# Total-RD/pymgrid

Measured on AMD Instinct MI355X. Metric: microgrid env-steps/sec, higher is better.
Workload: dtype f64

## Files before the change

pymgrid_amd/csrc/mgx_fused.hip:

```cpp
#include "mgx_kernels.hpp"

#ifndef MGX_FUSED_PART
#error "compile with -DMGX_FUSED_PART=<0..MGX_FUSED_PARTS-1>"
#endif

#if MGX_FUSED_PART == 0
#define MGX_PART_FLAGS(X) X(0) X(1) X(2) X(4)
#elif MGX_FUSED_PART == 1
#define MGX_PART_FLAGS(X) X(3) X(5)
#elif MGX_FUSED_PART == 2
#define MGX_PART_FLAGS(X) X(6) X(7)
#elif MGX_FUSED_PART == 3
#define MGX_PART_FLAGS(X) X(14)
#elif MGX_FUSED_PART == 4
#define MGX_PART_FLAGS(X) X(15)
#elif MGX_FUSED_PART == 5
#define MGX_PART_FLAGS(X)
#else
#error "MGX_FUSED_PART out of range"
#endif

#define MGX_CAT2(a, b) a##b
#define MGX_CAT(a, b) MGX_CAT2(a, b)

#if MGX_FUSED_PART == 5
namespace mgx {
#define MGX_STATIC_LAYOUTS(X) \
    X(7, 2, 2, 1, 1, 1) X(7, 2, 2, 2, 1, 1) X(7, 2, 2, 2, 2, 2) X(7, 1, 2, 1, 1, 1) X(7, 1, 2, 2, 1, 1) X(7, 2, 1, 1, 1, 1) X(7, 1, 1, 2, 1, 1) \
    X(3, 2, 2, 0, 1, 1) X(3, 2, 1, 0, 1, 1) X(3, 1, 2, 0, 1, 1) X(6, 0, 2, 1, 1, 1) X(6, 0, 2, 2, 1, 1) X(6, 0, 1, 2, 1, 1) \
                           \
    X(7, 3, 3, 1, 1, 1) X(7, 3, 2, 1, 1, 1) X(7, 2, 3, 1, 1, 1) X(3, 3, 3, 0, 1, 1) X(6, 0, 3, 1, 1, 1)
bool launch_step_k_multi_static(const MultiStaticLaunch &L)
{
#define X(FV, G, B, R, LD, PV)                                                                                                           \
    if (L.flags == FV && L.ng == G && L.nb == B && L.nr == R && L.nl == LD && L.np == PV) {                                             \
        using CT = CountsCT<G, B, R, LD, PV>;                                                                                          \
        step_k_multi_small_kernel<FV, CT, CT::slots><<<L.blocks, BLOCK_MULTI, 0, L.stream>>>(*L.k, L.actions, L.t, L.K, L.normalized, L.out); \
        return true;                                                                                                                    \
    }
    MGX_STATIC_LAYOUTS(X)
#undef X
    return false;
}
bool launch_rollout_multi_static(const MultiStaticRollout &L)
{
#define X(FV, G, B, R, LD, PV)                                                                                                           \
    if (L.flags == FV && L.ng == G && L.nb == B && L.nr == R && L.nl == LD && L.np == PV) {                                             \
        using CT = CountsCT<G, B, R, LD, PV>;                                                                                          \
        rollout_multi_small_kernel<FV, CT, CT::slots><<<L.blocks, BLOCK_MULTI, 0, L.stream>>>(*L.k, L.lists, L.n_lists, L.list_len,     \
                                                                                             L.ids, L.per_step, L.t, L.K, L.out);      \
        return true;                                                                                                                    \
    }
    MGX_STATIC_LAYOUTS(X)
#undef X
    return false;
}
}
#else

namespace mgx {

template <int F, bool RC, bool FC>
constexpr int ring_depth()
{
    if (FC) return RC ? ((F & F_GRID) ? 8 : MGX_RING_RICH) : MGX_RING;
    return (F & F_GRID) ? 4 : (RC ? 4 : MGX_RING);
}

template <int F>
static void step_k_dispatch(const FusedLaunch &L)
{
#define MGX_STEP_K(AT, RC, FC) step_k_kernel<F, ring_depth<F, RC, FC>(), AT, RC, FC><<<L.blocks, BLOCK_K, 0, L.stream>>>( \
        *L.k, (const AT *)L.actions, L.t, L.K, L.normalized, L.out, L.gpb)
    if (L.act_f32) {
        if (L.fact) { if (L.rich) MGX_STEP_K(float, true, true); else MGX_STEP_K(float, false, true); }
        else { if (L.rich) MGX_STEP_K(float, true, false); else MGX_STEP_K(float, false, false); }
    } else {
        if (L.fact) { if (L.rich) MGX_STEP_K(double, true, true); else MGX_STEP_K(double, false, true); }
        else { if (L.rich) MGX_STEP_K(double, true, false); else MGX_STEP_K(double, false, false); }
    }
#undef MGX_STEP_K
}

template <int F>
static void rollout_dispatch(const FusedLaunch &L)
{
#define MGX_ROLLOUT(PS, RC, FC) rollout_kernel<F, (F & F_GRID) ? 4 : MGX_RING_ROLLOUT, PS, RC, FC><<<L.blocks, BLOCK_K, 0, L.stream>>>( \
        *L.k, *L.tab, L.ids, L.t, L.K, L.out, L.gpb)
    if (L.fact) {
        if (L.per_step) { if (L.rich) MGX_ROLLOUT(true, true, true); else MGX_ROLLOUT(true, false, true); }
        else { if (L.rich) MGX_ROLLOUT(false, true, true); else MGX_ROLLOUT(false, false, true); }
    } else {
        if (L.per_step) { if (L.rich) MGX_ROLLOUT(true, true, false); else MGX_ROLLOUT(true, false, false); }
        else { if (L.rich) MGX_ROLLOUT(false, true, false); else MGX_ROLLOUT(false, false, false); }
    }
#undef MGX_ROLLOUT
}

bool MGX_CAT(launch_step_k_p, MGX_FUSED_PART)(const FusedLaunch &L)
{
    switch (L.flags) {
#define X(FV) case FV: step_k_dispatch<FV>(L); return true;
        MGX_PART_FLAGS(X)
#undef X
        default: return false;
    }
}

bool MGX_CAT(launch_rollout_p, MGX_FUSED_PART)(const FusedLaunch &L)
{
    switch (L.flags) {
#define X(FV) case FV: rollout_dispatch<FV>(L); return true;
        MGX_PART_FLAGS(X)
#undef X
        default: return false;
    }
}

}
#endif
```

pymgrid_amd/csrc/mgx_kernels.hpp:

```cpp
#pragma once
#include "mgx_core.hpp"

#include <type_traits>

namespace mgx {

#ifndef MGX_BLOCK
#define MGX_BLOCK 128
#endif
constexpr int BLOCK = MGX_BLOCK;
#ifndef MGX_RING
#define MGX_RING 8
#endif
#ifndef MGX_RING_RICH
#define MGX_RING_RICH 16
#endif
#ifndef MGX_BLOCK_K
#define MGX_BLOCK_K 256
#endif
constexpr int BLOCK_K = MGX_BLOCK_K;
#ifndef MGX_RING_ROLLOUT
#define MGX_RING_ROLLOUT 8
#endif

#ifndef MGX_HOT_NT
#define MGX_HOT_NT 1
#endif
#ifndef MGX_ACT_NT
#define MGX_ACT_NT 0
#endif
#ifndef MGX_OUT_NT
#define MGX_OUT_NT 0
#endif
#ifndef MGX_ROWS_NT
#define MGX_ROWS_NT 1
#endif
#ifndef MGX_STATE_NT
#define MGX_STATE_NT 1
#endif
#ifndef MGX_ROWS_TILE
#define MGX_ROWS_TILE 1
#endif
constexpr int ROW_TILE_MAX_D = 12;
__host__ __device__ inline bool step_rows_tiled(const KArgs &a, const void *obs)
{
    return MGX_ROWS_TILE && obs != nullptr && a.H == 0 && !a.obs_state_only && a.obs_dim <= ROW_TILE_MAX_D;
}

template <int F, typename OT>
__device__ __forceinline__ void observe_row_h0_tiled(const KArgs &a, int64_t i, int32_t t_next, const Params &p, const State &s,
                                                     OT *__restrict__ obs, int32_t pm, OT *tile)
{
    const int lane = threadIdx.x & 63;
    const int32_t D = a.obs_dim;
    observe_row_h0<F>(a, i, t_next, p, s, tile + lane * D, pm);
    __builtin_amdgcn_wave_barrier();
    typedef OT vec2 __attribute__((ext_vector_type(2)));
    typedef OT vec4 __attribute__((ext_vector_type(4)));
    OT *out = obs + (i - lane) * D;
    const int32_t total = 64 * D;
    if constexpr (sizeof(OT) == 8) {
        if ((reinterpret_cast<uintptr_t>(out) & 15) == 0) {
            for (int32_t e = 2 * lane; e < total; e += 128) {
                const vec2 v = *reinterpret_cast<const vec2 *>(tile + e);
#if MGX_ROWS_NT
                __builtin_nontemporal_store(v, reinterpret_cast<vec2 *>(out + e));
#else
                *reinterpret_cast<vec2 *>(out + e) = v;
#endif
            }
        } else {
            for (int32_t e = lane; e < total; e += 64) out[e] = tile[e];
        }
    } else {
        if ((total & 3) == 0 && (reinterpret_cast<uintptr_t>(out) & 15) == 0) {
            for (int32_t e = 4 * lane; e < total; e += 256) {
                const vec4 v = *reinterpret_cast<const vec4 *>(tile + e);
#if MGX_ROWS_NT
                __builtin_nontemporal_store(v, reinterpret_cast<vec4 *>(out + e));
#else
                *reinterpret_cast<vec4 *>(out + e) = v;
#endif
            }
        } else {
            for (int32_t e = 2 * lane; e < total; e += 128) {
                const vec2 v = *reinterpret_cast<const vec2 *>(tile + e);
                *reinterpret_cast<vec2 *>(out + e) = v;
            }
        }
    }
}

template <int F>
__device__ __forceinline__ void store_step_obs(const KArgs &a, void *__restrict__ obs, int64_t i, int32_t t_next, const Params &p,
                                               const State &s, int32_t pm = 0,
                                               double *tile = nullptr)
{
    constexpr int NSTATE = 4 * ((F & F_GENSET) != 0) + 2 * ((F & F_BATTERY) != 0);
// ... 92 lines not shown

template <int F, bool EP = false>
__global__ __launch_bounds__(BLOCK) void step_kernel(const KArgs a, const void *__restrict__ actions, int32_t t,
                                                     int normalized, double *__restrict__ reward,
                                                     uint8_t *__restrict__ done, void *__restrict__ obs,
                                                     double *__restrict__ log)
{
    t = resolve_t(a, t);
    extern __shared__ __attribute__((aligned(16))) double row_tiles[];
    const int64_t i = (int64_t)a.g0 + (int64_t)blockIdx.x * BLOCK + threadIdx.x;
    if (i < a.g1) step_body<F, EP>(a, actions, t, normalized, reward, done, obs, log, i, row_tiles + (threadIdx.x >> 6) * (64 * ROW_TILE_MAX_D));
    advance_counter_in_kernel(a, 1);
}

template <int F>
__global__ __launch_bounds__(BLOCK) void check_kernel(const KArgs a, const void *__restrict__ actions, int32_t t, int normalized,
                                                      uint32_t *__restrict__ violations)
{
    t = resolve_t(a, t);
    const int64_t i = (int64_t)a.g0 + (int64_t)blockIdx.x * BLOCK + threadIdx.x;
    if (i >= a.g1) return;
    Params p; State s; Inputs in; Outputs o; Derived d;
    load_state<F>(a.c, i, true, s);
    load_params<F>(a.c, i, p);
    derive<F>(p, d);
    const int64_t row = series_row(a, i, t);
    if (a.act_f32) load_inputs<F>(a.c, (const float *)actions, a.N, i, row, in, a.pm_pitch);
    else load_inputs<F>(a.c, (const double *)actions, a.N, i, row, in, a.pm_pitch);
    step_core<F>(p, d, s, in, normalized != 0, false, false, o);
    violations[i] = o.violations;
}

struct FusedOut {
    double *reward;
    uint8_t *done;
    double *soc_trace;
    uint32_t *status_trace;
    double *ret_acc;
    double *log;
};

template <typename AT>
struct RawInputs {
    AT a_goal, a_gen, a_bat, a_grid;
    double load, pv, g_pimp, g_pexp, g_co2, g_stat;
};

template <int F, typename AT>
__device__ __forceinline__ Inputs widen(const RawInputs<AT> &r)
{
    Inputs in;
    if constexpr (F & F_GENSET) { in.a_goal = (double)r.a_goal; in.a_gen = (double)r.a_gen; }
    if constexpr (F & F_BATTERY) in.a_bat = (double)r.a_bat;
    if constexpr (F & F_GRID) {
        in.a_grid = (double)r.a_grid;
        in.g_pimp = r.g_pimp; in.g_pexp = r.g_pexp; in.g_co2 = r.g_co2; in.g_stat = r.g_stat;
    }
    in.load = r.load; in.pv = r.pv;
    return in;
}

template <int F, typename AT>
__device__ __forceinline__ void load_inputs_at(const AT *__restrict__ act, const double *__restrict__ lts,
                                               const double *__restrict__ pts, const double *__restrict__ gts,
                                               int64_t N, int64_t i, int64_t off, RawInputs<AT> &in)
{
    constexpr int A = 2 * ((F & F_GENSET) != 0) + ((F & F_BATTERY) != 0) + ((F & F_GRID) != 0);
    const AT *a = act + off * A;
    int k = 0;
    if constexpr (F & F_GENSET) { in.a_goal = a[k]; in.a_gen = a[k + 1]; k += 2; }
    if constexpr (F & F_BATTERY) { in.a_bat = a[k]; k += 1; }
    if constexpr (F & F_GRID) { in.a_grid = a[k]; k += 1; }
    in.load = lts[off];
    in.pv = pts[off];
    if constexpr (F & F_GRID) {
        const double *g = gts + (4 * off - 3 * i);
        in.g_pimp = g[0]; in.g_pexp = g[N]; in.g_co2 = g[2 * N]; in.g_stat = g[3 * N];
    }
}

#ifndef MGX_FACT_ROWS
#define MGX_FACT_ROWS 128
#endif
constexpr int FACT_ROWS = MGX_FACT_ROWS;

template <int F>
__device__ __forceinline__ void stage_base_rows(const mgx_columns &c, int64_t row0, int32_t n, double *lds, int nthreads)
{
    const int32_t cnt = n * PP;
    const double *__restrict__ bl = c.base_load + row0 * PP;
    const double *__restrict__ bp = c.base_pv + row0 * PP;
    for (int32_t j = threadIdx.x; j < cnt; j += nthreads) {
        lds[j] = bl[j];
        lds[FACT_ROWS * PP + j] = bp[j];
        if constexpr (F & F_GRID) lds[2 * FACT_ROWS * PP + j] = c.base_co2[row0 * PP + j];
    }
}

struct BaseVals { double load, pv, co2; };

template <int F>
__device__ __forceinline__ BaseVals read_base_row(const double *lds, int32_t r, const GridFactors &f)
{
    BaseVals b;
    b.load = lds[r * PP + f.lp];
    b.pv = lds[FACT_ROWS * PP + r * PP + f.pp];
    b.co2 = 0.0;
    if constexpr (F & F_GRID) b.co2 = lds[2 * FACT_ROWS * PP + r * PP + f.cp];
    return b;
}

struct OutageWords {
    uint64_t cur, nxt;
    int64_t wi;
};

__device__ __forceinline__ void outage_init(const mgx_columns &c, int64_t N, int64_t i, int32_t T, int32_t t0, OutageWords &w)
{
    w.wi = t0 >> 6; w.cur = 0; w.nxt = 0;
    if (c.outage_bits) {
        w.cur = c.outage_bits[w.wi * N + i];
        if ((w.wi + 1) * 64 < T) w.nxt = c.outage_bits[(w.wi + 1) * N + i];
    }
}

__device__ __forceinline__ double outage_status(const mgx_columns &c, int64_t N, int64_t i, int32_t T, int32_t row, bool first,
                                                OutageWords &w)
{
    if (!first && (row & 63) == 0) {
        w.cur = w.nxt; w.wi += 1; w.nxt = 0;
        if (c.outage_bits && (w.wi + 1) * 64 < T) w.nxt = c.outage_bits[(w.wi + 1) * N + i];
    }
    return ((w.cur >> (row & 63)) & 1ull) ? 0.0 : 1.0;
}

template <typename AT>
struct RawActions {
    AT a_goal, a_gen, a_bat, a_grid;
};

template <int F, typename AT>
__device__ __forceinline__ void load_actions_at(const AT *__restrict__ row, uint32_t i32, RawActions<AT> &r)
{
    constexpr int A = 2 * ((F & F_GENSET) != 0) + ((F & F_BATTERY) != 0) + ((F & F_GRID) != 0);
    const AT *a = row + i32 * (uint32_t)A;
    int k = 0;
#if MGX_ACT_NT
    if constexpr (F & F_GENSET) { r.a_goal = __builtin_nontemporal_load(a + k); r.a_gen = __builtin_nontemporal_load(a + k + 1); k += 2; }
    if constexpr (F & F_BATTERY) { r.a_bat = __builtin_nontemporal_load(a + k); k += 1; }
    if constexpr (F & F_GRID) { r.a_grid = __builtin_nontemporal_load(a + k); k += 1; }
#else
    if constexpr (F & F_GENSET) { r.a_goal = a[k]; r.a_gen = a[k + 1]; k += 2; }
    if constexpr (F & F_BATTERY) { r.a_bat = a[k]; k += 1; }
    if constexpr (F & F_GRID) { r.a_grid = a[k]; k += 1; }
#endif
}

__device__ __forceinline__ void store_done(const KArgs &a, uint8_t *__restrict__ done, int64_t off, int64_t i, int32_t k, bool dn)
{
    if (a.done_bits) {
        const unsigned long long b = __ballot(dn);
        const int lane = threadIdx.x & 63;
        if ((lane & 15) == 0) {
            const int64_t W = ((int64_t)a.N + 15) >> 4;
            reinterpret_cast<uint16_t *>(done)[(int64_t)k * W + (i >> 4)] = (uint16_t)(b >> (lane & 48));
        }
    } else {
        done[off] = (uint8_t)dn;
    }
}

template <int F, int U, typename AT, bool RICH, bool FACT>
__global__ __launch_bounds__(BLOCK_K) void step_k_kernel(const KArgs a, const AT *__restrict__ actions, int32_t t0,
                                                         int32_t K, int normalized, const FusedOut out_rt, int32_t gpb)
{
    FusedOut out = out_rt;
    if constexpr (!RICH) { out.log = nullptr; out.status_trace = nullptr; }
    const int32_t K_launch = K;
    t0 = resolve_t(a, t0);
    K = resolve_k(a, t0, K);
    const int64_t i = (int64_t)a.g0 + (int64_t)blockIdx.x * gpb + threadIdx.x;
    const bool active = (int32_t)threadIdx.x < gpb && i < a.g1;
    if constexpr (!FACT) { if (!active) return; }
    const int64_t N = a.N;
    constexpr int A_DIM = 2 * ((F & F_GENSET) != 0) + ((F & F_BATTERY) != 0) + ((F & F_GRID) != 0);
    Params p; State s; Derived d;
    const bool norm = normalized != 0;
    const bool want_soc = (out.soc_trace != nullptr) || (out.log != nullptr);
    bool gen_instant = false;
    int32_t k_done = 0;
    if (active) {
        load_state<F>(a.c, i, out.log != nullptr, s);
        load_params<F>(a.c, i, p);
        derive<F>(p, d);
        gen_instant = genset_wave_is_instant<F>(p, s);
        k_done = (a.grid_final ? a.grid_final[i] : a.final_step) - 1 - t0;
    }
    double ret = 0.0;

    const bool hot = !RICH && out.reward != nullptr && out.done == nullptr && (!(F & F_BATTERY) || out.soc_trace != nullptr) &&
                     a.shaper == MGX_SHAPER_NONE;
    const uint32_t i32 = (uint32_t)i;
    auto consume = [&](auto gi_tag, auto hot_tag, const Inputs &in, int32_t k, int64_t off) __attribute__((always_inline)) {
        constexpr bool GI = decltype(gi_tag)::value, HOT = decltype(hot_tag)::value;
        Outputs o;
        step_core<F>(p, d, s, in, norm, HOT ? (F & F_BATTERY) != 0 : want_soc, GI, o);
        if constexpr (HOT) {
            const double r = o.reward;
#if MGX_HOT_NT
            __builtin_nontemporal_store(r, (out.reward + (int64_t)k * N) + i32);
            if constexpr (F & F_BATTERY) __builtin_nontemporal_store(s.soc, (out.soc_trace + (int64_t)k * N) + i32);
#else
            (out.reward + (int64_t)k * N)[i32] = r;
            if constexpr (F & F_BATTERY) (out.soc_trace + (int64_t)k * N)[i32] = s.soc;
#endif
            ret += r;
            return;
        }
        const double r = shaped_reward<F>(a.shaper, o);
        {
#if MGX_OUT_NT
            if (out.reward) __builtin_nontemporal_store(r, out.reward + off);
            if (out.done) store_done(a, out.done, off, i, k, k >= k_done);
            if constexpr (F & F_BATTERY) { if (out.soc_trace) __builtin_nontemporal_store(s.soc, out.soc_trace + off); }
            if constexpr (F & F_GENSET) { if (out.status_trace) __builtin_nontemporal_store(s.status, out.status_trace + off); }
#else
            if (out.reward) out.reward[off] = r;
            if (out.done) store_done(a, out.done, off, i, k, k >= k_done);
            if constexpr (F & F_BATTERY) { if (out.soc_trace) out.soc_trace[off] = s.soc; }
            if constexpr (F & F_GENSET) { if (out.status_trace) out.status_trace[off] = s.status; }
#endif
            if (out.log) store_log<F>(out.log + (off - i) * a.log_dim + i, N, o, s.status);
        }
        ret += r;
    };
    auto specialised = [&](auto fn) __attribute__((always_inline)) {
        if constexpr ((F & F_GENSET) != 0) {
            if (gen_instant) { if (hot) fn(std::true_type{}, std::true_type{}); else fn(std::true_type{}, std::false_type{}); }
            else { if (hot) fn(std::false_type{}, std::true_type{}); else fn(std::false_type{}, std::false_type{}); }
        } else {
            if (hot) fn(std::false_type{}, std::true_type{}); else fn(std::false_type{}, std::false_type{});
        }
    };

    if constexpr (FACT) {
        __shared__ double base_lds[((F & F_GRID) ? 3 : 2) * FACT_ROWS * PP];
        static_assert(FACT_ROWS % U == 0, "ring slots are addressed by k % U across LDS chunks");
        GridFactors f;
        f.lr = 0.0; f.pr = 0.0; f.lp = 0u; f.pp = 0u; f.cp = 0u; f.pat = 0u;
        OutageWords ow;
        ow.cur = 0; ow.nxt = 0; ow.wi = 0;
        RawActions<AT> ring[U];
        if (active) {
            load_factors<F>(a.c, i, f);
            if constexpr (F & F_GRID) outage_init(a.c, N, i, a.T, t0, ow);
#pragma unroll
            for (int u = 0; u < U; u++)
                if (u < K) load_actions_at<F>(actions + (int64_t)u * N * A_DIM, i32, ring[u]);
        }
        int64_t off = i;
        auto run_chunk = [&](auto gi_tag, auto hot_tag, int32_t kb, int32_t n) __attribute__((always_inline)) {
            BaseVals nb = read_base_row<F>(base_lds, 0, f);
            for (int32_t k0 = kb; k0 < kb + n; k0 += U) {
#pragma unroll
                for (int u = 0; u < U; u++) {
                    const int32_t k = k0 + u;
                    if (k < kb + n) {
                        const RawActions<AT> ra = ring[u];
                        if (k + U < K) load_actions_at<F>(actions + (int64_t)(k + U) * N * A_DIM, i32, ring[u]);
                        Inputs in;
                        if constexpr (F & F_GENSET) { in.a_goal = (double)ra.a_goal; in.a_gen = (double)ra.a_gen; }
                        if constexpr (F & F_BATTERY) in.a_bat = (double)ra.a_bat;
                        in.load = fact_load(nb.load, f.lr);
                        in.pv = fact_pv(nb.pv, f.pr);
                        if constexpr (F & F_GRID) {
                            in.a_grid = (double)ra.a_grid;
                            in.g_pimp = tariff_price((int32_t)f.pat, t0 + k); in.g_pexp = 0.0;
                            in.g_co2 = nb.co2;
                            in.g_stat = outage_status(a.c, N, i, a.T, t0 + k, k == 0, ow);
                        }
                        const int32_t rn = (k + 1 - kb < n) ? k + 1 - kb : n - 1;
                        nb = read_base_row<F>(base_lds, rn, f);
                        consume(gi_tag, hot_tag, in, k, off);
                        off += N;
                    }
                }
            }
        };
        for (int32_t kb = 0; kb < K; kb += FACT_ROWS) {
            const int32_t n = K - kb < FACT_ROWS ? K - kb : FACT_ROWS;
            __syncthreads();
            stage_base_rows<F>(a.c, (int64_t)t0 + kb, n, base_lds, BLOCK_K);
            __syncthreads();
            if (active) specialised([&](auto gi_tag, auto hot_tag) __attribute__((always_inline)) { run_chunk(gi_tag, hot_tag, kb, n); });
        }
        if (!active) return;
    } else {
        const double *__restrict__ lts = a.c.load_ts + (int64_t)t0 * N;
        const double *__restrict__ pts = a.c.pv_ts + (int64_t)t0 * N;
        const double *__restrict__ gts = (F & F_GRID) ? a.c.grid_ts + (int64_t)t0 * 4 * N : nullptr;
        specialised([&](auto gi_tag, auto hot_tag) __attribute__((always_inline)) {
            RawInputs<AT> ring[U];
#pragma unroll
            for (int u = 0; u < U; u++)
                if (u < K) load_inputs_at<F>(actions, lts, pts, gts, N, i, (int64_t)u * N + i, ring[u]);

            int64_t off = i;
            for (int32_t k0 = 0; k0 < K; k0 += U) {
#pragma unroll
                for (int u = 0; u < U; u++) {
                    const int32_t k = k0 + u;
                    if (k < K) {
                        const Inputs in = widen<F>(ring[u]);
                        if (k + U < K) load_inputs_at<F>(actions, lts, pts, gts, N, i, off + (int64_t)U * N, ring[u]);
                        consume(gi_tag, hot_tag, in, k, off);
                        off += N;
                    }
                }
            }
        });
    }
    if constexpr (F & F_BATTERY) { if (!want_soc) s.soc = s.charge / p.bat_cmax; }
    store_state<F>(a.c, i, s);
    if (out.ret_acc) out.ret_acc[i] += ret;
    advance_counter_in_kernel(a, K_launch);
}

struct FusedLaunch {
    int flags;
    bool act_f32, rich, fact, per_step;
    unsigned blocks;
    hipStream_t stream;
    const KArgs *k;
    const void *actions;
    const PLWords *tab;
    const uint8_t *ids;
    int32_t t, K;
    int normalized;
    FusedOut out;
    int32_t gpb;
};
constexpr int MGX_FUSED_PARTS = 6;
struct MultiStaticLaunch {
    int flags, ng, nb, nr, nl, np;
    unsigned blocks;
    hipStream_t stream;
    const KArgs *k;
    const void *actions;
    int32_t t, K;
    int normalized;
    FusedOut out;
};
bool launch_step_k_multi_static(const MultiStaticLaunch &L);
struct MultiStaticRollout {
    int flags, ng, nb, nr, nl, np;
    unsigned blocks;
    hipStream_t stream;
    const KArgs *k;
    const int32_t *lists;
    int32_t n_lists, list_len;
    const int32_t *ids;
    int per_step;
    int32_t t, K;
    FusedOut out;
};
bool launch_rollout_multi_static(const MultiStaticRollout &L);
bool launch_step_k_p0(const FusedLaunch &L); bool launch_step_k_p1(const FusedLaunch &L); bool launch_step_k_p2(const FusedLaunch &L);
bool launch_step_k_p3(const FusedLaunch &L); bool launch_step_k_p4(const FusedLaunch &L);
bool launch_rollout_p0(const FusedLaunch &L); bool launch_rollout_p1(const FusedLaunch &L); bool launch_rollout_p2(const FusedLaunch &L);
bool launch_rollout_p3(const FusedLaunch &L); bool launch_rollout_p4(const FusedLaunch &L);
enum : int { EP_SRC_FACT = 0, EP_SRC_GRID_MAJOR = 1, EP_SRC_GATHER = 2 };
struct EpisodeLaunch {
    int flags;
    int src;
    bool per_step;
    unsigned blocks;
    int32_t gpb;
    hipStream_t stream;
    const KArgs *k;
    const KArgs *k_dev;
    const PLWords *tab;
    const uint8_t *ids;
    int32_t t, K;
    FusedOut out;
    mgx_episode_stats stats;
};
constexpr int MGX_EPISODE_PARTS = 2;
bool launch_rollout_episodes_p0(const EpisodeLaunch &L); bool launch_rollout_episodes_p1(const EpisodeLaunch &L);
struct StepEpisodeLaunch {
    int flags;
    int src;
    bool act_f32;
    unsigned blocks;
    int32_t gpb;
    hipStream_t stream;
    const KArgs *k;
    const KArgs *k_dev;
    const void *actions;
    int32_t t, K;
    int normalized;
    FusedOut out;
    mgx_episode_stats stats;
};
constexpr int MGX_STEP_EPISODE_PARTS = 2;
bool launch_step_k_episodes_p0(const StepEpisodeLaunch &L); bool launch_step_k_episodes_p1(const StepEpisodeLaunch &L);

template <int F>
__global__ __launch_bounds__(BLOCK) void observe_kernel(const KArgs a, int32_t t, void *__restrict__ obs)
{
    t = resolve_t_obs(a, t);
    const int64_t i = (int64_t)a.g0 + (int64_t)blockIdx.x * BLOCK + threadIdx.x;
    if (i >= a.g1) return;
    Params p; State s;
    load_state<F>(a.c, i, true, s);
    load_params<F>(a.c, i, p);
    store_step_obs<F>(a, obs, i, t + (a.ep_off ? a.ep_off[i] : 0), p, s, a.pm_pitch);
}

struct WindowPlan {
    int32_t grid_col_base;
    int32_t ld;
    int32_t group;
};

// ... 746 lines not shown
            MGX_FLEET_V_DISCRETE(0, EPV) MGX_FLEET_V_DISCRETE(1, EPV) MGX_FLEET_V_DISCRETE(2, EPV) MGX_FLEET_V_DISCRETE(3, EPV)       \
            MGX_FLEET_V_DISCRETE(4, EPV) MGX_FLEET_V_DISCRETE(5, EPV) MGX_FLEET_V_DISCRETE(6, EPV) MGX_FLEET_V_DISCRETE(7, EPV)       \
            MGX_FLEET_V_DISCRETE(14, EPV)                                                                                             \
            default: { step_discrete_body<15, EPV>(B.k, *hd.tab, (const int32_t *)B.actions, hd.t, nullptr, B.reward, B.done, B.obs, B.log, i); } break; \
        }                                                                                                                             \
        return;                                                                                                                       \
    }                                                                                                                                 \
    switch (hd.flags) {                                                                                                               \
        MGX_FLEET_V_STEP(0, EPV) MGX_FLEET_V_STEP(1, EPV) MGX_FLEET_V_STEP(2, EPV) MGX_FLEET_V_STEP(3, EPV) MGX_FLEET_V_STEP(4, EPV)   \
        MGX_FLEET_V_STEP(5, EPV) MGX_FLEET_V_STEP(6, EPV) MGX_FLEET_V_STEP(7, EPV) MGX_FLEET_V_STEP(14, EPV)                          \
        default: { step_body<15, EPV>(B.k, B.actions, hd.t, normalized, B.reward, B.done, B.obs, B.log, i); } break;                  \
    }

template <bool EP>
static __global__ __launch_bounds__(BLOCK) void fleet_step_kernel_v(const FleetArgsV fa)
{
    MGX_FLEET_V_HEAD
    MGX_FLEET_V_SWITCHES(EP)
}

template <int F, int U, bool PER_STEP, bool RICH, bool FACT>
__global__ __launch_bounds__(BLOCK_K) void rollout_kernel(const KArgs a, const PLWords tab, const uint8_t *__restrict__ ids,
                                                          int32_t t0, int32_t K, const FusedOut out_rt, int32_t gpb)
{
    FusedOut out = out_rt;
    if constexpr (!RICH) { out.log = nullptr; out.status_trace = nullptr; }
    const int32_t K_launch = K;
    t0 = resolve_t(a, t0);
    K = resolve_k(a, t0, K);
    const int64_t i = (int64_t)a.g0 + (int64_t)blockIdx.x * gpb + threadIdx.x;
    const bool active = (int32_t)threadIdx.x < gpb && i < a.g1;
    if constexpr (!FACT) { if (!active) return; }
    const int64_t N = a.N;
    Params p; State s; Derived d;
    const bool want_soc = (out.soc_trace != nullptr) || (out.log != nullptr);
    bool gen_instant = false;
    int32_t k_done = 0;
    uint32_t word = 0u;
    if (active) {
        load_state<F>(a.c, i, out.log != nullptr, s);
        load_params<F>(a.c, i, p);
        derive<F>(p, d);
        gen_instant = genset_wave_is_instant<F>(p, s);
        k_done = (a.grid_final ? a.grid_final[i] : a.final_step) - 1 - t0;
        word = PER_STEP ? 0u : pl_select(tab, ids[i]);
    }
    double ret = 0.0;

    const bool hot = !RICH && out.reward != nullptr && out.done == nullptr && (!(F & F_BATTERY) || out.soc_trace != nullptr) &&
                     a.shaper == MGX_SHAPER_NONE;
    const uint32_t i32 = (uint32_t)i;
    auto consume = [&](auto gi_tag, auto hot_tag, Inputs &in, int32_t k, int64_t off) __attribute__((always_inline)) {
        constexpr bool GI = decltype(gi_tag)::value, HOT = decltype(hot_tag)::value;
        double bat_q;
        uint32_t xv = 0u;
        populate_core<F, RICH>(p, s, word, in, bat_q, 0.0 + -1 * in.load, in.pv, GI, &xv);
        Outputs o;
        step_core<F, true>(p, d, s, in, false, HOT ? (F & F_BATTERY) != 0 : want_soc, GI, o, bat_q);
        if constexpr (RICH) o.violations |= xv;
        if constexpr (HOT) {
            const double r = o.reward;
            (out.reward + (int64_t)k * N)[i32] = r;
            if constexpr (F & F_BATTERY) (out.soc_trace + (int64_t)k * N)[i32] = s.soc;
            ret += r;
            return;
        }
        const double r = shaped_reward<F>(a.shaper, o);
        if (out.reward) out.reward[off] = r;
        if (out.done) store_done(a, out.done, off, i, k, k >= k_done);
        if constexpr (F & F_BATTERY) { if (out.soc_trace) out.soc_trace[off] = s.soc; }
        if constexpr (F & F_GENSET) { if (out.status_trace) out.status_trace[off] = s.status; }
        if (out.log) store_log<F>(out.log + (off - i) * a.log_dim + i, N, o, s.status);
        ret += r;
    };
    auto specialised = [&](auto fn) __attribute__((always_inline)) {
        if constexpr ((F & F_GENSET) != 0) {
            if (gen_instant) { if (hot) fn(std::true_type{}, std::true_type{}); else fn(std::true_type{}, std::false_type{}); }
            else { if (hot) fn(std::false_type{}, std::true_type{}); else fn(std::false_type{}, std::false_type{}); }
        } else {
            if (hot) fn(std::false_type{}, std::true_type{}); else fn(std::false_type{}, std::false_type{});
        }
    };
    if constexpr (FACT) {
        __shared__ double base_lds[((F & F_GRID) ? 3 : 2) * FACT_ROWS * PP];
        static_assert(FACT_ROWS % U == 0, "ring slots are addressed by k % U across LDS chunks");
        GridFactors f;
        f.lr = 0.0; f.pr = 0.0; f.lp = 0u; f.pp = 0u; f.cp = 0u; f.pat = 0u;
        OutageWords ow;
        ow.cur = 0; ow.nxt = 0; ow.wi = 0;
        static_assert(U <= 8, "the id ring is one 64-bit register");
        uint64_t idq = 0;
        if (active) {
            load_factors<F>(a.c, i, f);
            if constexpr (F & F_GRID) outage_init(a.c, N, i, a.T, t0, ow);
            if constexpr (PER_STEP) {
#pragma unroll
                for (int u = 0; u < U; u++)
                    if (u < K) idq |= (uint64_t)(ids + (int64_t)u * N)[i32] << (8 * u);
            }
        }
        int64_t off = i;
        auto run_chunk = [&](auto gi_tag, auto hot_tag, int32_t kb, int32_t n) __attribute__((always_inline)) {
            BaseVals nb = read_base_row<F>(base_lds, 0, f);
            for (int32_t k0 = kb; k0 < kb + n; k0 += U) {
#pragma unroll
                for (int u = 0; u < U; u++) {
                    const int32_t k = k0 + u;
                    if (k < kb + n) {
                        if constexpr (PER_STEP) {
                            word = pl_select(tab, (int32_t)((idq >> (8 * u)) & 0xffu));
                            if (k + U < K)
                                idq = (idq & ~(0xffull << (8 * u))) | ((uint64_t)(ids + (int64_t)(k + U) * N)[i32] << (8 * u));
                        }
                        Inputs in;
                        in.load = fact_load(nb.load, f.lr);
                        in.pv = fact_pv(nb.pv, f.pr);
                        in.g_stat = 1.0;
                        if constexpr (F & F_GRID) {
                            in.g_pimp = tariff_price((int32_t)f.pat, t0 + k); in.g_pexp = 0.0;
                            in.g_co2 = nb.co2;
                            in.g_stat = outage_status(a.c, N, i, a.T, t0 + k, k == 0, ow);
                        }
                        const int32_t rn = (k + 1 - kb < n) ? k + 1 - kb : n - 1;
                        nb = read_base_row<F>(base_lds, rn, f);
                        consume(gi_tag, hot_tag, in, k, off);
                        off += N;
                    }
                }
            }
        };
        for (int32_t kb = 0; kb < K; kb += FACT_ROWS) {
            const int32_t n = K - kb < FACT_ROWS ? K - kb : FACT_ROWS;
            __syncthreads();
            stage_base_rows<F>(a.c, (int64_t)t0 + kb, n, base_lds, BLOCK_K);
            __syncthreads();
            if (active) specialised([&](auto gi_tag, auto hot_tag) __attribute__((always_inline)) { run_chunk(gi_tag, hot_tag, kb, n); });
        }
        if (!active) return;
    } else {
        specialised([&](auto gi_tag, auto hot_tag) __attribute__((always_inline)) {
            const double *__restrict__ lts = a.c.load_ts + (int64_t)t0 * N;
            const double *__restrict__ pts = a.c.pv_ts + (int64_t)t0 * N;
            const double *__restrict__ gts = (F & F_GRID) ? a.c.grid_ts + (int64_t)t0 * 4 * N : nullptr;
            Inputs ring[U];
            uint8_t idr[U];
#pragma unroll
            for (int u = 0; u < U; u++)
                if (u < K) {
                    load_series_at<F>(lts, pts, gts, N, i, (int64_t)u * N + i, ring[u]);
                    if constexpr (PER_STEP) idr[u] = ids[(int64_t)u * N + i];
                }

            int64_t off = i;
            for (int32_t k0 = 0; k0 < K; k0 += U) {
#pragma unroll
                for (int u = 0; u < U; u++) {
                    const int32_t k = k0 + u;
                    if (k < K) {
                        Inputs in = ring[u];
                        if constexpr (PER_STEP) word = pl_select(tab, idr[u]);
                        if (k + U < K) {
                            load_series_at<F>(lts, pts, gts, N, i, off + (int64_t)U * N, ring[u]);
                            if constexpr (PER_STEP) idr[u] = ids[off + (int64_t)U * N];
                        }
                        consume(gi_tag, hot_tag, in, k, off);
                        off += N;
                    }
                }
            }
        });
    }
    if constexpr (F & F_BATTERY) { if (!want_soc) s.soc = s.charge / p.bat_cmax; }
    store_state<F>(a.c, i, s);
    if (out.ret_acc) out.ret_acc[i] += ret;
    advance_counter_in_kernel(a, K_launch);
}

constexpr int BLOCK_MULTI = 64;

__device__ __forceinline__ StepLists multi_lists(const KArgs &a, double *lds)
{
    const int cap = multi_list_capacity(a.n_load, a.n_pv, a.n_genset, a.n_battery, a.n_grid);
    StepLists L;
    L.stride = BLOCK_MULTI; L.n_prov = 0; L.n_absb = 0;
    L.prov = lds + threadIdx.x;
    L.absb = lds + (size_t)cap * BLOCK_MULTI + threadIdx.x;
    return L;
}

template <typename OT>
__device__ __forceinline__ void observe_series_multi(const double *__restrict__ ts, int64_t row_stride, int32_t T, int32_t t, int32_t H,
                                                     double lo, double hi, OT *__restrict__ obs, int obs_stride = 1, bool noisy = false,
                                                     double noise_std = 0.0, uint64_t noise_seed = 0, int noise_increase = 0,
                                                     int64_t grid = 0, uint32_t comp = 0)
{
    const double fill = (hi + lo) / 2, sp = space_spread(lo, hi);
    for (int h = 0; h <= H; h++) {
        const bool in = t < T && t + h < T;
        double v = in ? ts[(int64_t)(t + h) * row_stride] : 0.0;
        if (noisy && in && h > 0) {
            const double sd = noise_increase ? noise_std * (1.0 + log(1.0 + (double)(h - 1))) : noise_std;
            v += sd * forecast_normal(noise_seed, grid, comp, t, h);
        }
        obs[h * obs_stride] = (OT)obs_series_value(v, in, h > 0, lo, hi, fill, sp);
    }
}

template <int F, typename OT>
__device__ inline void observe_state_multi(const KArgs &a, int64_t i, OT *__restrict__ dst, int64_t stride)
{
    const int64_t N = a.N;
    int64_t k = 0;
    if constexpr (F & F_GENSET) {
        for (int j = 0; j < a.n_genset; j++) {
            const int64_t c = (int64_t)j * N + i;
            const uint32_t times = a.c.gen_times[c], st = a.c.gen_status[c];
            const double su = (double)(times & 0xff), wd = (double)((times >> 16) & 0xff);
// ... 1050 lines not shown
```

pymgrid_amd/_lib.py:

```python
import ctypes as C
import json
import os
import re
import subprocess
import sys

_PKG = os.path.dirname(os.path.abspath(__file__))
_ROOT = os.path.dirname(_PKG)
LIB_PATH = os.environ.get("MGX_LIB") or os.path.join(_PKG, "libmgx.so")
SOURCES = [os.path.join(_PKG, "csrc", f) for f in ("mgx_abi.hip", "mgx_fused.hip", "mgx_kernels.hpp", "mgx_core.hpp", "mgx_episodes.hip",
                                                      "mgx_step_episodes.hip")] + \
          [os.path.join(_ROOT, "include", "mgx.h")]
FUSED_PARTS = 6
EPISODE_PARTS = 2
STEP_EPISODE_PARTS = 2

HIPCC_FLAGS = ["--offload-arch=gfx950", "-O3", "-std=c++17", "-ffp-contract=off", "-fno-fast-math", "-fPIC"]

MGX_OK, MGX_ERR_INVALID, MGX_ERR_UNSUPPORTED, MGX_ERR_RANGE, MGX_ERR_DEVICE = range(5)
V_GENSET_RANGE, V_BATTERY_LIMIT, V_GRID_LIMIT, V_GENSET_GOAL, V_GENSET_NEGATIVE, V_NEGATIVE_LIMIT = 1, 2, 4, 8, 16, 32
V_EXPAND_CONSUME, V_EXPAND_PRODUCE, V_EXPAND_SIGN = 64, 128, 256
V_EXPAND = V_EXPAND_CONSUME | V_EXPAND_PRODUCE | V_EXPAND_SIGN
V_ASSERTS = V_GENSET_GOAL | V_GENSET_NEGATIVE | V_NEGATIVE_LIMIT | V_EXPAND
ABI_VERSION = 9
# ... 200 lines not shown
    return os.path.exists(path) and built_hash(path) == source_hash()


def build(force=False, verbose=False, defs=(), lib_path=None, abi_only=False):
    if lib_path is not None or defs:
        return _build(lib_path or LIB_PATH, list(defs), verbose, os.path.basename(lib_path or "variant") + ".o", abi_only=abi_only)
    if os.environ.get("MGX_LIB") and os.path.exists(LIB_PATH) and not force:
        return LIB_PATH
    if not force and up_to_date(LIB_PATH):
        return LIB_PATH
    return _build(LIB_PATH, [], verbose, "", force)


def _build(LIB_PATH, extra_defs, verbose, objtag, force=True, abi_only=False):
    import fcntl
    with open(LIB_PATH + ".lock", "w") as lock:
        fcntl.flock(lock, fcntl.LOCK_EX)
        try:
            if not force and not extra_defs and up_to_date(LIB_PATH):
                return LIB_PATH
            stamp = source_hash(extra_defs)
            hipcc = os.environ.get("HIPCC", "/opt/rocm/bin/hipcc")
            tmp = f"{LIB_PATH}.{os.getpid()}.tmp"
            objdir = os.path.join(_PKG, "csrc", "_build" + ("_" + objtag if objtag else ""))
            os.makedirs(objdir, exist_ok=True)
            units = [(SOURCES[0], [], os.path.join(objdir, "mgx_abi.o"))] + \
                    [(SOURCES[1], [f"-DMGX_FUSED_PART={p}"], os.path.join(objdir, f"mgx_fused_{p}.o")) for p in range(FUSED_PARTS)] + \
                    [(SOURCES[4], [f"-DMGX_EPISODE_PART={p}"], os.path.join(objdir, f"mgx_episodes_{p}.o")) for p in range(EPISODE_PARTS)] + \
                    [(SOURCES[5], [f"-DMGX_STEP_EPISODE_PART={p}"], os.path.join(objdir, f"mgx_step_episodes_{p}.o")) for p in range(STEP_EPISODE_PARTS)]
            if abi_only:
                base = os.path.join(_PKG, "csrc", "_build")
                fused = [os.path.join(base, f"mgx_fused_{p}.o") for p in range(FUSED_PARTS)] + \
                        [os.path.join(base, f"mgx_episodes_{p}.o") for p in range(EPISODE_PARTS)] + \
                        [os.path.join(base, f"mgx_step_episodes_{p}.o") for p in range(STEP_EPISODE_PARTS)]
                if not all(os.path.exists(f) for f in fused):
                    raise FileNotFoundError("abi_only variants link the product build's mgx_fused objects: build() first")
                units = units[:1]
            procs = []
            for src, defs, obj in units:
                cmd = [hipcc] + HIPCC_FLAGS + ["-Rpass-analysis=kernel-resource-usage"] + defs + extra_defs + ["-c", src, "-o", obj]
                if verbose:
                    print(" ".join(cmd))
                procs.append((cmd, subprocess.Popen(cmd, stderr=subprocess.PIPE, text=True)))
            usage = {}
            for cmd, p in procs:
                _, err = p.communicate()
                if p.returncode != 0:
                    sys.stderr.write(err)
                    for _, q in procs:
                        if q.poll() is None:
                            q.kill()
                    raise subprocess.CalledProcessError(p.returncode, cmd)
                usage.update(_parse_resource_usage(err))
                rest = "\n".join(ln for ln in err.splitlines() if "kernel-resource-usage" not in ln and not _REMARK_ECHO.match(ln))
                if rest.strip() and verbose:
                    sys.stderr.write(rest + "\n")
            with open(os.path.join(objdir, "resource_usage.json"), "w") as fh:
                json.dump(usage, fh, indent=0, sort_keys=True)
            link = [hipcc, "--offload-arch=gfx950", "-fPIC", "-shared"] + [obj for _, _, obj in units] + (fused if abi_only else []) + ["-o", tmp]
            if verbose:
                print(" ".join(link))
            subprocess.run(link, check=True)
            os.replace(tmp, LIB_PATH)
            with open(LIB_PATH + ".srchash.tmp", "w") as fh:
                fh.write(stamp + "\n")
            os.replace(LIB_PATH + ".srchash.tmp", LIB_PATH + ".srchash")
        finally:
            fcntl.flock(lock, fcntl.LOCK_UN)
    return LIB_PATH


_REMARK_ECHO = re.compile(r"^\s*(\d+ \||\||In file included from)")


def _parse_resource_usage(stderr_text):
    out, cur = {}, None
    for ln in stderr_text.splitlines():
        m = re.search(r"remark:\s+Function Name: (\S+)", ln)
        if m:
            cur = out.setdefault(m.group(1), {})
            continue
        if cur is None:
            continue
        for key, pat in (("sgpr", r"TotalSGPRs: (\d+)"), ("vgpr", r"remark:\s+VGPRs: (\d+)"), ("scratch", r"ScratchSize \[bytes/lane\]: (\d+)"),
                         ("lds", r"LDS Size \[bytes/block\]: (\d+)"), ("sgpr_spill", r"SGPRs Spill: (\d+)"), ("vgpr_spill", r"VGPRs Spill: (\d+)")):
            m = re.search(pat, ln)
            if m:
                cur[key] = int(m.group(1))
    if out:
        try:
            names = list(out)
            dem = subprocess.run(["c++filt"], input="\n".join(names), capture_output=True, text=True).stdout.split("\n")
            out = {(d.split("(")[0].replace("void ", "") or n): out[n] for n, d in zip(names, dem)}
        except OSError:
            pass
    return out


def resource_usage():
    f = os.path.join(_PKG, "csrc", "_build", "resource_usage.json")
    try:
        with open(f) as fh:
            return json.load(fh)
    except (OSError, ValueError):
        return None


_lib = None


def lib():
    global _lib
    if _lib is None:
        if not os.path.exists(LIB_PATH):
            raise ImportError(f"{LIB_PATH} is missing: build it with __graft_entry__.build() "
                              f"(pymgrid_amd has no CPU fallback)")
        L = C.CDLL(LIB_PATH)
        for name, (res, args) in SYMBOLS.items():
            fn = getattr(L, name)
            fn.restype, fn.argtypes = res, args
        if L.mgx_abi_version() != ABI_VERSION:
            raise ImportError(f"libmgx.so ABI {L.mgx_abi_version()} != binding ABI {ABI_VERSION}; rebuild")
        assert C.sizeof(Layout) == 64
        _lib = L
    return _lib


def check(rc):
    if rc != MGX_OK:
        raise MgxError(rc, lib().mgx_last_error().decode())


def set_tunable(name, value):
    check(lib().mgx_set_tunable(TUNABLES.index(name), int(value)))


def get_tunable(name):
    v, d = C.c_int64(), C.c_int64()
    check(lib().mgx_get_tunable(TUNABLES.index(name), C.byref(v), C.byref(d)))
    return v.value, d.value
```

Measured before the change: 134.6 billion.

## Add unguarded whole-group factorised step_k path with deeper action ring

Adds a specialised step_k kernel variant for non-grid flags, used when K is a multiple of the ring depth and the lean hot output path applies. It removes the per-step bounds checks, refills the action ring right after each consume, and uses a ring depth of 16. FACT_ROWS becomes a per-depth template constant so the LDS chunking stays aligned to the ring. The cost is more register pressure from the deeper ring, an extra kernel instantiation, and a raw waitcnt intrinsic.

```diff
diff --git a/pymgrid_amd/csrc/mgx_fused.hip b/pymgrid_amd/csrc/mgx_fused.hip
--- a/pymgrid_amd/csrc/mgx_fused.hip
+++ b/pymgrid_amd/csrc/mgx_fused.hip
@@ -68,8 +68,24 @@
 }
 
 template <int F>
+constexpr int whole_depth()
+{
+    return (F & F_GRID) ? 0 : MGX_RING_WHOLE;
+}
+
+template <int F>
 static void step_k_dispatch(const FusedLaunch &L)
 {
+    if constexpr (whole_depth<F>() > 0) {
+        constexpr int UW = whole_depth<F>();
+        if (step_k_whole_launch<F>(L, UW)) {
+            if (L.act_f32) step_k_kernel<F, UW, WholeGroups<float>, false, true><<<L.blocks, BLOCK_K, 0, L.stream>>>(
+                               *L.k, (const float *)L.actions, L.t, L.K, L.normalized, L.out, L.gpb);
+            else step_k_kernel<F, UW, WholeGroups<double>, false, true><<<L.blocks, BLOCK_K, 0, L.stream>>>(
+                     *L.k, (const double *)L.actions, L.t, L.K, L.normalized, L.out, L.gpb);
+            return;
+        }
+    }
 #define MGX_STEP_K(AT, RC, FC) step_k_kernel<F, ring_depth<F, RC, FC>(), AT, RC, FC><<<L.blocks, BLOCK_K, 0, L.stream>>>( \
         *L.k, (const AT *)L.actions, L.t, L.K, L.normalized, L.out, L.gpb)
     if (L.act_f32) {
diff --git a/pymgrid_amd/csrc/mgx_kernels.hpp b/pymgrid_amd/csrc/mgx_kernels.hpp
--- a/pymgrid_amd/csrc/mgx_kernels.hpp
+++ b/pymgrid_amd/csrc/mgx_kernels.hpp
@@ -14,6 +14,9 @@
 #endif
 #ifndef MGX_RING_RICH
 #define MGX_RING_RICH 16
+#endif
+#ifndef MGX_RING_WHOLE
+#define MGX_RING_WHOLE 16
 #endif
 #ifndef MGX_BLOCK_K
 #define MGX_BLOCK_K 256
@@ -272,9 +275,14 @@
 #ifndef MGX_FACT_ROWS
 #define MGX_FACT_ROWS 128
 #endif
-constexpr int FACT_ROWS = MGX_FACT_ROWS;
-
-template <int F>
+template <int U>
+constexpr int fact_rows()
+{
+    static_assert(U >= 1 && U <= MGX_FACT_ROWS, "ring depth out of range");
+    return MGX_FACT_ROWS / U * U;
+}
+
+template <int F, int ROWS>
 __device__ __forceinline__ void stage_base_rows(const mgx_columns &c, int64_t row0, int32_t n, double *lds, int nthreads)
 {
     const int32_t cnt = n * PP;
@@ -282,21 +290,21 @@
     const double *__restrict__ bp = c.base_pv + row0 * PP;
     for (int32_t j = threadIdx.x; j < cnt; j += nthreads) {
         lds[j] = bl[j];
-        lds[FACT_ROWS * PP + j] = bp[j];
-        if constexpr (F & F_GRID) lds[2 * FACT_ROWS * PP + j] = c.base_co2[row0 * PP + j];
+        lds[ROWS * PP + j] = bp[j];
+        if constexpr (F & F_GRID) lds[2 * ROWS * PP + j] = c.base_co2[row0 * PP + j];
     }
 }
 
 struct BaseVals { double load, pv, co2; };
 
-template <int F>
+template <int F, int ROWS>
 __device__ __forceinline__ BaseVals read_base_row(const double *lds, int32_t r, const GridFactors &f)
 {
     BaseVals b;
     b.load = lds[r * PP + f.lp];
-    b.pv = lds[FACT_ROWS * PP + r * PP + f.pp];
+    b.pv = lds[ROWS * PP + r * PP + f.pp];
     b.co2 = 0.0;
-    if constexpr (F & F_GRID) b.co2 = lds[2 * FACT_ROWS * PP + r * PP + f.cp];
+    if constexpr (F & F_GRID) b.co2 = lds[2 * ROWS * PP + r * PP + f.cp];
     return b;
 }
 
@@ -360,10 +368,19 @@
     }
 }
 
-template <int F, int U, typename AT, bool RICH, bool FACT>
-__global__ __launch_bounds__(BLOCK_K) void step_k_kernel(const KArgs a, const AT *__restrict__ actions, int32_t t0,
+template <typename T>
+struct WholeGroups {};
+template <typename ATAG>
+struct StepKActions { using type = ATAG; static constexpr bool whole = false; };
+template <typename T>
+struct StepKActions<WholeGroups<T>> { using type = T; static constexpr bool whole = true; };
+
+template <int F, int U, typename ATAG, bool RICH, bool FACT>
+__global__ __launch_bounds__(BLOCK_K) void step_k_kernel(const KArgs a, const typename StepKActions<ATAG>::type *__restrict__ actions, int32_t t0,
                                                          int32_t K, int normalized, const FusedOut out_rt, int32_t gpb)
 {
+    using AT = typename StepKActions<ATAG>::type;
+    constexpr bool WHOLE = StepKActions<ATAG>::whole;
     FusedOut out = out_rt;
     if constexpr (!RICH) { out.log = nullptr; out.status_trace = nullptr; }
     const int32_t K_launch = K;
@@ -425,7 +442,10 @@
         ret += r;
     };
     auto specialised = [&](auto fn) __attribute__((always_inline)) {
-        if constexpr ((F & F_GENSET) != 0) {
+        if constexpr (WHOLE) {
+            if constexpr ((F & F_GENSET) != 0) { if (gen_instant) fn(std::true_type{}, std::true_type{}); else fn(std::false_type{}, std::true_type{}); }
+            else fn(std::false_type{}, std::true_type{});
+        } else if constexpr ((F & F_GENSET) != 0) {
             if (gen_instant) { if (hot) fn(std::true_type{}, std::true_type{}); else fn(std::true_type{}, std::false_type{}); }
             else { if (hot) fn(std::false_type{}, std::true_type{}); else fn(std::false_type{}, std::false_type{}); }
         } else {
@@ -434,6 +454,7 @@
     };
 
     if constexpr (FACT) {
+        constexpr int FACT_ROWS = fact_rows<U>();
         __shared__ double base_lds[((F & F_GRID) ? 3 : 2) * FACT_ROWS * PP];
         static_assert(FACT_ROWS % U == 0, "ring slots are addressed by k % U across LDS chunks");
         GridFactors f;
@@ -446,11 +467,44 @@
             if constexpr (F & F_GRID) outage_init(a.c, N, i, a.T, t0, ow);
 #pragma unroll
             for (int u = 0; u < U; u++)
-                if (u < K) load_actions_at<F>(actions + (int64_t)u * N * A_DIM, i32, ring[u]);
+                if (WHOLE || u < K) load_actions_at<F>(actions + (int64_t)u * N * A_DIM, i32, ring[u]);
         }
         int64_t off = i;
+        static_assert(!WHOLE || (FACT && !RICH), "the unguarded form exists for the lean factorised loop");
         auto run_chunk = [&](auto gi_tag, auto hot_tag, int32_t kb, int32_t n) __attribute__((always_inline)) {
-            BaseVals nb = read_base_row<F>(base_lds, 0, f);
+            BaseVals nb = read_base_row<F, FACT_ROWS>(base_lds, 0, f);
+            if constexpr (WHOLE) {
+                auto run_group = [&](auto refill_tag, int32_t k0) __attribute__((always_inline)) {
+#pragma unroll
+                    for (int u = 0; u < U; u++) {
+                        const int32_t k = k0 + u;
+                        const RawActions<AT> ra = ring[u];
+                        Inputs in;
+                        if constexpr (F & F_GENSET) { in.a_goal = (double)ra.a_goal; in.a_gen = (double)ra.a_gen; }
+                        if constexpr (F & F_BATTERY) in.a_bat = (double)ra.a_bat;
+                        in.load = fact_load(nb.load, f.lr);
+                        in.pv = fact_pv(nb.pv, f.pr);
+                        if constexpr (F & F_GRID) {
+                            in.a_grid = (double)ra.a_grid;
+                            in.g_pimp = tariff_price((int32_t)f.pat, t0 + k); in.g_pexp = 0.0;
+                            in.g_co2 = nb.co2;
+                            in.g_stat = outage_status(a.c, N, i, a.T, t0 + k, k == 0, ow);
+                        }
+                        int32_t rn = k + 1 - kb;
+                        if (u == U - 1 && rn == n) rn = n - 1;
+                        nb = read_base_row<F, FACT_ROWS>(base_lds, rn, f);
+                        consume(gi_tag, hot_tag, in, k, off);
+                        if constexpr (decltype(refill_tag)::value) load_actions_at<F>(actions + (int64_t)(k + U) * N * A_DIM, i32, ring[u]);
+                        off += N;
+                    }
+                };
+                const int32_t ke = kb + n, kr = ke < K ? ke : ke - U;
+                int32_t k0 = kb;
+                __builtin_amdgcn_s_waitcnt(0x0F70);
+                for (; k0 < kr; k0 += U) run_group(std::true_type{}, k0);
+                if (k0 < ke) run_group(std::false_type{}, k0);
+                return;
+            }
             for (int32_t k0 = kb; k0 < kb + n; k0 += U) {
 #pragma unroll
                 for (int u = 0; u < U; u++) {
@@ -470,7 +524,7 @@
                             in.g_stat = outage_status(a.c, N, i, a.T, t0 + k, k == 0, ow);
                         }
                         const int32_t rn = (k + 1 - kb < n) ? k + 1 - kb : n - 1;
-                        nb = read_base_row<F>(base_lds, rn, f);
+                        nb = read_base_row<F, FACT_ROWS>(base_lds, rn, f);
                         consume(gi_tag, hot_tag, in, k, off);
                         off += N;
                     }
@@ -480,7 +534,7 @@
         for (int32_t kb = 0; kb < K; kb += FACT_ROWS) {
             const int32_t n = K - kb < FACT_ROWS ? K - kb : FACT_ROWS;
             __syncthreads();
-            stage_base_rows<F>(a.c, (int64_t)t0 + kb, n, base_lds, BLOCK_K);
+            stage_base_rows<F, FACT_ROWS>(a.c, (int64_t)t0 + kb, n, base_lds, BLOCK_K);
             __syncthreads();
             if (active) specialised([&](auto gi_tag, auto hot_tag) __attribute__((always_inline)) { run_chunk(gi_tag, hot_tag, kb, n); });
         }
@@ -530,6 +584,13 @@
     FusedOut out;
     int32_t gpb;
 };
+template <int F>
+inline bool step_k_whole_launch(const FusedLaunch &L, int U)
+{
+    const bool hot = !L.rich && L.out.reward != nullptr && L.out.done == nullptr && (!(F & F_BATTERY) || L.out.soc_trace != nullptr) &&
+                     L.k->shaper == MGX_SHAPER_NONE;
+    return L.fact && hot && L.K % U == 0 && L.k->t_dev == nullptr;
+}
 constexpr int MGX_FUSED_PARTS = 6;
 struct MultiStaticLaunch {
     int flags, ng, nb, nr, nl, np;
@@ -1442,6 +1503,7 @@
         }
     };
     if constexpr (FACT) {
+        constexpr int FACT_ROWS = fact_rows<U>();
         __shared__ double base_lds[((F & F_GRID) ? 3 : 2) * FACT_ROWS * PP];
         static_assert(FACT_ROWS % U == 0, "ring slots are addressed by k % U across LDS chunks");
         GridFactors f;
@@ -1461,7 +1523,7 @@
         }
         int64_t off = i;
         auto run_chunk = [&](auto gi_tag, auto hot_tag, int32_t kb, int32_t n) __attribute__((always_inline)) {
-            BaseVals nb = read_base_row<F>(base_lds, 0, f);
+            BaseVals nb = read_base_row<F, FACT_ROWS>(base_lds, 0, f);
             for (int32_t k0 = kb; k0 < kb + n; k0 += U) {
 #pragma unroll
                 for (int u = 0; u < U; u++) {
@@ -1482,7 +1544,7 @@
                             in.g_stat = outage_status(a.c, N, i, a.T, t0 + k, k == 0, ow);
                         }
                         const int32_t rn = (k + 1 - kb < n) ? k + 1 - kb : n - 1;
-                        nb = read_base_row<F>(base_lds, rn, f);
+                        nb = read_base_row<F, FACT_ROWS>(base_lds, rn, f);
                         consume(gi_tag, hot_tag, in, k, off);
                         off += N;
                     }
@@ -1492,7 +1554,7 @@
         for (int32_t kb = 0; kb < K; kb += FACT_ROWS) {
             const int32_t n = K - kb < FACT_ROWS ? K - kb : FACT_ROWS;
             __syncthreads();
-            stage_base_rows<F>(a.c, (int64_t)t0 + kb, n, base_lds, BLOCK_K);
+            stage_base_rows<F, FACT_ROWS>(a.c, (int64_t)t0 + kb, n, base_lds, BLOCK_K);
             __syncthreads();
             if (active) specialised([&](auto gi_tag, auto hot_tag) __attribute__((always_inline)) { run_chunk(gi_tag, hot_tag, kb, n); });
         }
```

Result: faster. 136.2 billion, median of 5 (+1.2%).

## Add steady-state unrolled group with hoisted action normalization in factored hot path

Applied to the files above, without the earlier changes.

Adds a steady-state loop for the factored hot path that handles full groups of U steps without bounds checks. Actions are denormalized inline and step_core is called with normalization off, and the normalize flag is made a compile-time constant when there is no grid component. Empty asm barriers order the prefetch address computation after the action conversions. This targets per-step branch overhead and the runtime normalize branch, at the cost of more code paths and higher register pressure. It also moves the grid input code into a shared helper and adds AGPR parsing to the resource report.

```diff
diff --git a/pymgrid_amd/_lib.py b/pymgrid_amd/_lib.py
--- a/pymgrid_amd/_lib.py
+++ b/pymgrid_amd/_lib.py
@@ -306,7 +306,7 @@
             continue
         if cur is None:
             continue
-        for key, pat in (("sgpr", r"TotalSGPRs: (\d+)"), ("vgpr", r"remark:\s+VGPRs: (\d+)"), ("scratch", r"ScratchSize \[bytes/lane\]: (\d+)"),
+        for key, pat in (("sgpr", r"TotalSGPRs: (\d+)"), ("vgpr", r"remark:\s+VGPRs: (\d+)"), ("agpr", r"remark:\s+AGPRs: (\d+)"), ("scratch", r"ScratchSize \[bytes/lane\]: (\d+)"),
                          ("lds", r"LDS Size \[bytes/block\]: (\d+)"), ("sgpr_spill", r"SGPRs Spill: (\d+)"), ("vgpr_spill", r"VGPRs Spill: (\d+)")):
             m = re.search(pat, ln)
             if m:
diff --git a/pymgrid_amd/csrc/mgx_kernels.hpp b/pymgrid_amd/csrc/mgx_kernels.hpp
--- a/pymgrid_amd/csrc/mgx_kernels.hpp
+++ b/pymgrid_amd/csrc/mgx_kernels.hpp
@@ -14,6 +14,9 @@
 #endif
 #ifndef MGX_RING_RICH
 #define MGX_RING_RICH 16
+#endif
+#ifndef MGX_STEADY_NORM_CT
+#define MGX_STEADY_NORM_CT 1
 #endif
 #ifndef MGX_BLOCK_K
 #define MGX_BLOCK_K 256
@@ -391,10 +394,10 @@
     const bool hot = !RICH && out.reward != nullptr && out.done == nullptr && (!(F & F_BATTERY) || out.soc_trace != nullptr) &&
                      a.shaper == MGX_SHAPER_NONE;
     const uint32_t i32 = (uint32_t)i;
-    auto consume = [&](auto gi_tag, auto hot_tag, const Inputs &in, int32_t k, int64_t off) __attribute__((always_inline)) {
+    auto consume = [&](auto gi_tag, auto hot_tag, const Inputs &in, int32_t k, int64_t off, bool nrm) __attribute__((always_inline)) {
         constexpr bool GI = decltype(gi_tag)::value, HOT = decltype(hot_tag)::value;
         Outputs o;
-        step_core<F>(p, d, s, in, norm, HOT ? (F & F_BATTERY) != 0 : want_soc, GI, o);
+        step_core<F>(p, d, s, in, nrm, HOT ? (F & F_BATTERY) != 0 : want_soc, GI, o);
         if constexpr (HOT) {
             const double r = o.reward;
 #if MGX_HOT_NT
@@ -449,9 +452,56 @@
                 if (u < K) load_actions_at<F>(actions + (int64_t)u * N * A_DIM, i32, ring[u]);
         }
         int64_t off = i;
+        auto series_inputs = [&](Inputs &in, BaseVals &nb, int32_t k, int32_t kb, int32_t n) __attribute__((always_inline)) {
+            in.load = fact_load(nb.load, f.lr);
+            in.pv = fact_pv(nb.pv, f.pr);
+            if constexpr (F & F_GRID) {
+                in.g_pimp = tariff_price((int32_t)f.pat, t0 + k); in.g_pexp = 0.0;
+                in.g_co2 = nb.co2;
+                in.g_stat = outage_status(a.c, N, i, a.T, t0 + k, k == 0, ow);
+            }
+            const int32_t rn = (k + 1 - kb < n) ? k + 1 - kb : n - 1;
+            nb = read_base_row<F>(base_lds, rn, f);
+        };
+        auto steady_group = [&](auto gi_tag, auto hot_tag, auto nrm, BaseVals &nb, int32_t k0, int32_t kb, int32_t n) __attribute__((always_inline)) {
+            const bool NORM = nrm;
+            auto take = [&](AT v, double sp, double lo) __attribute__((always_inline)) -> double {
+                return NORM ? lo + sp * (double)v : (double)v;
+            };
+            uint64_t lane_b = (uint64_t)(i32 * (uint32_t)A_DIM) * sizeof(AT);
+#pragma unroll
+            for (int u = 0; u < U; u++) {
+                const int32_t k = k0 + u;
+                Inputs in;
+                if constexpr (F & F_GENSET) {
+                    in.a_goal = (double)ring[u].a_goal > 0.5 ? 1.0 : 0.0;
+                    in.a_gen = take(ring[u].a_gen, d.gen_sp, 0.0);
+                }
+                if constexpr (F & F_BATTERY) in.a_bat = take(ring[u].a_bat, d.bat_sp, d.bat_lo);
+                if constexpr (F & F_GRID) in.a_grid = take(ring[u].a_grid, d.grid_sp, d.grid_lo);
+                if constexpr (F & F_GENSET) asm("" : "+v"(lane_b) : "v"(in.a_gen));
+                if constexpr (F & F_BATTERY) asm("" : "+v"(lane_b) : "v"(in.a_bat));
+                if constexpr (F & F_GRID) asm("" : "+v"(lane_b) : "v"(in.a_grid));
+                load_actions_at<F>(reinterpret_cast<const AT *>(reinterpret_cast<const char *>(actions + (int64_t)(k + U) * N * A_DIM) + lane_b), 0u, ring[u]);
+                series_inputs(in, nb, k, kb, n);
+                consume(gi_tag, hot_tag, in, k, off, false);
+                off += N;
+            }
+        };
         auto run_chunk = [&](auto gi_tag, auto hot_tag, int32_t kb, int32_t n) __attribute__((always_inline)) {
             BaseVals nb = read_base_row<F>(base_lds, 0, f);
-            for (int32_t k0 = kb; k0 < kb + n; k0 += U) {
+            int32_t k0 = kb;
+            if constexpr (!RICH && decltype(hot_tag)::value) {
+                constexpr bool NORM_CT = MGX_STEADY_NORM_CT && !(F & F_GRID);
+                if (NORM_CT && norm) {
+                    for (; k0 + U <= kb + n && k0 + 2 * U <= K; k0 += U) steady_group(gi_tag, hot_tag, std::true_type{}, nb, k0, kb, n);
+                } else if (NORM_CT) {
+                    for (; k0 + U <= kb + n && k0 + 2 * U <= K; k0 += U) steady_group(gi_tag, hot_tag, std::false_type{}, nb, k0, kb, n);
+                } else {
+                    for (; k0 + U <= kb + n && k0 + 2 * U <= K; k0 += U) steady_group(gi_tag, hot_tag, norm, nb, k0, kb, n);
+                }
+            }
+            for (; k0 < kb + n; k0 += U) {
 #pragma unroll
                 for (int u = 0; u < U; u++) {
                     const int32_t k = k0 + u;
@@ -461,17 +511,9 @@
                         Inputs in;
                         if constexpr (F & F_GENSET) { in.a_goal = (double)ra.a_goal; in.a_gen = (double)ra.a_gen; }
                         if constexpr (F & F_BATTERY) in.a_bat = (double)ra.a_bat;
-                        in.load = fact_load(nb.load, f.lr);
-                        in.pv = fact_pv(nb.pv, f.pr);
-                        if constexpr (F & F_GRID) {
-                            in.a_grid = (double)ra.a_grid;
-                            in.g_pimp = tariff_price((int32_t)f.pat, t0 + k); in.g_pexp = 0.0;
-                            in.g_co2 = nb.co2;
-                            in.g_stat = outage_status(a.c, N, i, a.T, t0 + k, k == 0, ow);
-                        }
-                        const int32_t rn = (k + 1 - kb < n) ? k + 1 - kb : n - 1;
-                        nb = read_base_row<F>(base_lds, rn, f);
-                        consume(gi_tag, hot_tag, in, k, off);
+                        if constexpr (F & F_GRID) in.a_grid = (double)ra.a_grid;
+                        series_inputs(in, nb, k, kb, n);
+                        consume(gi_tag, hot_tag, in, k, off, norm);
                         off += N;
                     }
                 }
@@ -503,7 +545,7 @@
                     if (k < K) {
                         const Inputs in = widen<F>(ring[u]);
                         if (k + U < K) load_inputs_at<F>(actions, lts, pts, gts, N, i, off + (int64_t)U * N, ring[u]);
-                        consume(gi_tag, hot_tag, in, k, off);
+                        consume(gi_tag, hot_tag, in, k, off, norm);
                         off += N;
                     }
                 }
```

Measured after the change: 133.5 billion before, 134.5 billion after (median of 6 runs). About the same (+0.8%).
